# Farofeiro231/LiDAR_SLAM

Measured on AMD Instinct MI355X. Metric: scans/sec (RANSAC+UKF, 720-pt scans) at 1/2/4/8 MI355X + HBM GB/s vs peak, higher is better.
Workload: dtype f64; 1 GPU; C3: 4096 synthetic 720-pt scans per GPU, chunked 7x100+20; RANSAC (100 trials, 20 mm, mt19937 hypotheses) + landmark association + UKF predict/update (n=3, L=20); scans_per_gpu=4096, trials=100, landmarks=20, hyp=mt19937, parallelism=dp1 (scan shards, no collective)

## Files before the change

lidar_slam_amd/csrc/lslam_ctx.h:

```cpp
#pragma once
#include "lslam_hazards.h"

constexpr int LSLAM_EV_RING = 64;
constexpr int NSLOTS = 2;

static thread_local std::string g_err;

static size_t default_steps_budget() { return (size_t)2 << 30; }

static size_t default_reloc_budget() {
    if (const char *e = getenv("LSLAM_RELOC_BUDGET")) {
        const long long v = atoll(e);
        if (v > 0) return (size_t)v;
    }
    return (size_t)4096 * 41 * 21 * 21 * 4;
}

static int set_err(int code, const char *msg) {
    g_err = msg;
    return code;
}

#define HIPCHK(expr)                                                                  \
    do {                                                                              \
        hipError_t _e = (expr);                                                       \
        if (_e != hipSuccess) {                                                       \
            g_err = std::string(#expr) + ": " + hipGetErrorString(_e);                \
            return LSLAM_ERR_HIP;                                                     \
        }                                                                             \
    } while (0)

struct DevBuf {
    void *p = nullptr;
    size_t bytes = 0;
    template <typename T>
    T *as() const { return (T *)p; }
    hipError_t release() {
        void *q = p;
        p = nullptr;
        bytes = 0;
        return q ? hipFree(q) : hipSuccess;
    }
    static bool fits(const DevBuf *b, int n, size_t need) {
        for (int i = 0; i < n; i++)
            if (b[i].bytes < need) return false;
        return true;
    }
    static int ensure(lslam_ctx *c, DevBuf *b, int n, size_t need, const char *what);
    int ensure(lslam_ctx *c, size_t need, const char *what) { return ensure(c, this, 1, need, what); }
};

struct lslam_ctx {
    int device = 0;
    hipStream_t stream = nullptr;
    bool timing = false;
    hipEvent_t ev0[LSLAM_K_COUNT][LSLAM_EV_RING] = {}, ev1[LSLAM_K_COUNT][LSLAM_EV_RING] = {};
    int head[LSLAM_K_COUNT] = {}, npend[LSLAM_K_COUNT] = {};
    double total_ms[LSLAM_K_COUNT] = {};
    int64_t launches[LSLAM_K_COUNT] = {};
    DevBuf scr;
    DevBuf escr;
    DevBuf cscr;
    DevBuf mscr;
    DevBuf rscr;
    size_t reloc_budget = default_reloc_budget();
    int resolve_beside = 0;
    int n_cus = 1;
    uint32_t timing_mask = 0xffffffffu;
    uint32_t *rt_all = nullptr;
    DevBuf seedst[3];
    hipStream_t sstream = nullptr;
    hipEvent_t ev_seeded[2] = {};
    hipEvent_t ev_seed_read[2] = {};
    int seed_next = 0;
    DevBuf cutb[4];
    int cut_next = 0;
    size_t steps_budget = default_steps_budget();
    hipStream_t pstream = nullptr;
    DevBuf pslot[NSLOTS];
    int next_slot = 0;
    hipEvent_t ev_slot_free[NSLOTS] = {};
    hipEvent_t ev_produced = nullptr;
    hipEvent_t ev_copy = nullptr;
    hipEvent_t ev_call = nullptr;
    hipStream_t ustream = nullptr;
    hipEvent_t ev_ukf = nullptr;
    HazardState hz;
    int prev_slot = 0;
    DevBuf spec_dirty[2];
    int spec_cur = 0;
};

int DevBuf::ensure(lslam_ctx *c, DevBuf *b, int n, size_t need, const char *what) {
    if (fits(b, n, need)) return LSLAM_OK;
    for (hipStream_t s : {c->stream, c->pstream, c->ustream, c->sstream}) HIPCHK(hipStreamSynchronize(s));
    for (int i = 0; i < n; i++) HIPCHK(b[i].release());
    for (int i = 0; i < n; i++) {
        const hipError_t e = hipMalloc(&b[i].p, need);
        if (e == hipErrorOutOfMemory) {
            g_err = std::string("hipMalloc: out of memory (") + what + ")";
            return LSLAM_ERR_NOMEM;
        }
        HIPCHK(e);
        b[i].bytes = need;
    }
    return LSLAM_OK;
}

static const std::vector<uint32_t> &reject_tables() {
    static const std::vector<uint32_t> t = [] {
        std::vector<uint32_t> v((size_t)(RT_KMAX - 1) * RT_DWORDS);
        for (uint32_t K = 2; K <= RT_KMAX; K++)
            for (uint32_t r = 0; r < (uint32_t)RT_ROWS; r++)
                for (uint32_t q = 0; q < (uint32_t)RT_ST; q++)
                    v[(size_t)(K - 2) * RT_DWORDS + r * RT_ST + q] = rt_word(K, r, q);
        return v;
    }();
    return t;
}

static int ctx_init(lslam_ctx *c, int device) {
    c->device = device;
    HIPCHK(hipDeviceGetAttribute(&c->n_cus, hipDeviceAttributeMultiprocessorCount, device));
    if (c->n_cus < 1) c->n_cus = 1;
    if (const char *e = getenv("LSLAM_MT_SPECULATE")) c->hz.speculate = atoi(e) != 0;
    HIPCHK(hipStreamCreateWithFlags(&c->stream, hipStreamNonBlocking));
    for (int k = 0; k < LSLAM_K_COUNT; k++)
        for (int r = 0; r < LSLAM_EV_RING; r++) {
            HIPCHK(hipEventCreate(&c->ev0[k][r]));
            HIPCHK(hipEventCreate(&c->ev1[k][r]));
        }
    {
        int lo_pri = 0, hi_pri = 0;
        if (hipDeviceGetStreamPriorityRange(&lo_pri, &hi_pri) != hipSuccess) hi_pri = 0;
        HIPCHK(hipStreamCreateWithPriority(&c->pstream, hipStreamNonBlocking, hi_pri));
    }
    HIPCHK(hipStreamCreateWithFlags(&c->sstream, hipStreamNonBlocking));
    for (int i = 0; i < 2; i++) {
        HIPCHK(hipEventCreateWithFlags(&c->ev_seeded[i], hipEventDisableTiming));
        HIPCHK(hipEventCreateWithFlags(&c->ev_seed_read[i], hipEventDisableTiming));
        HIPCHK(hipEventRecord(c->ev_seed_read[i], c->stream));
    }
    for (int i = 0; i < NSLOTS; i++) HIPCHK(hipEventCreateWithFlags(&c->ev_slot_free[i], hipEventDisableTiming));
    HIPCHK(hipEventCreateWithFlags(&c->ev_produced, hipEventDisableTiming));
    HIPCHK(hipStreamCreateWithFlags(&c->ustream, hipStreamNonBlocking));
    HIPCHK(hipEventCreateWithFlags(&c->ev_ukf, hipEventDisableTiming));
    HIPCHK(hipEventCreateWithFlags(&c->ev_copy, hipEventDisableTiming));
    HIPCHK(hipEventCreateWithFlags(&c->ev_call, hipEventDisableTiming));
    for (int i = 0; i < NSLOTS; i++) HIPCHK(hipEventRecord(c->ev_slot_free[i], c->stream));
    HIPCHK(hipEventRecord(c->ev_copy, c->stream));
    HIPCHK(hipEventRecord(c->ev_call, c->stream));
    const std::vector<uint32_t> &t = reject_tables();
    HIPCHK(hipMalloc(&c->rt_all, t.size() * 4));
    HIPCHK(hipMemcpy(c->rt_all, t.data(), t.size() * 4, hipMemcpyHostToDevice));
    return LSLAM_OK;
}

extern "C" {

#define LSLAM_STR_(x) #x
#define LSLAM_STR(x) LSLAM_STR_(x)
#ifndef LSLAM_SRC_HASH
#define LSLAM_SRC_HASH "0000000000000000"
#endif
const char *lslam_version(void) {
    return "lidarslam-mi355x 0.3.0 (abi " LSLAM_STR(LSLAM_ABI_VERSION) ", src " LSLAM_SRC_HASH ", gfx950)";
}

const char *lslam_status_string(int st) {
    switch (st) {
        case LSLAM_OK: return "ok";
        case LSLAM_ERR_ARG: return "invalid argument";
        case LSLAM_ERR_HIP: return "HIP runtime error";
        case LSLAM_ERR_NOMEM: return "out of memory";
        case LSLAM_ERR_CAPACITY: return "capacity exceeded";
        case LSLAM_ERR_UNSUPPORTED: return "unsupported";
        default: return "unknown status";
    }
}

const char *lslam_last_error(void) { return g_err.c_str(); }

int lslam_device_count(int *n) {
    if (!n) return LSLAM_ERR_ARG;
    int c = 0;
    hipError_t e = hipGetDeviceCount(&c);
    if (e != hipSuccess) c = 0;
    *n = c;
    return LSLAM_OK;
}

int lslam_ctx_create(int device, lslam_ctx **out) {
    if (!out) return LSLAM_ERR_ARG;
    *out = nullptr;
    int n = 0;
    HIPCHK(hipGetDeviceCount(&n));
    if (device < 0 || device >= n) return set_err(LSLAM_ERR_ARG, "device index out of range");
    HIPCHK(hipSetDevice(device));
    lslam_ctx *c = new (std::nothrow) lslam_ctx();
    if (!c) return LSLAM_ERR_NOMEM;
    const int st = ctx_init(c, device);
    if (st) {
        lslam_ctx_destroy(c);
        return st;
    }
    *out = c;
    return LSLAM_OK;
}

int lslam_ctx_destroy(lslam_ctx *c) {
    if (!c) return LSLAM_OK;
    (void)hipSetDevice(c->device);
    hipStream_t streams[4] = {c->stream, c->pstream, c->ustream, c->sstream};
    for (hipStream_t s : streams)
        if (s) (void)hipStreamSynchronize(s);
    for (int k = 0; k < LSLAM_K_COUNT; k++)
        for (int r = 0; r < LSLAM_EV_RING; r++) {
            if (c->ev0[k][r]) (void)hipEventDestroy(c->ev0[k][r]);
            if (c->ev1[k][r]) (void)hipEventDestroy(c->ev1[k][r]);
        }
    for (DevBuf *b : {&c->scr, &c->escr, &c->cscr, &c->mscr, &c->rscr}) (void)b->release();
    for (DevBuf &b : c->seedst) (void)b.release();
    for (DevBuf &b : c->cutb) (void)b.release();
    for (DevBuf &b : c->pslot) (void)b.release();
    for (DevBuf &b : c->spec_dirty) (void)b.release();
    if (c->rt_all) (void)hipFree(c->rt_all);
    hipEvent_t evs[10] = {c->ev_seeded[0], c->ev_seeded[1], c->ev_seed_read[0], c->ev_seed_read[1], c->ev_slot_free[0],
                          c->ev_slot_free[1], c->ev_produced, c->ev_copy, c->ev_call, c->ev_ukf};
    for (hipEvent_t e : evs)
        if (e) (void)hipEventDestroy(e);
    for (hipStream_t s : streams)
        if (s) (void)hipStreamDestroy(s);
    delete c;
    return LSLAM_OK;
}

int lslam_sync(lslam_ctx *c) {
    if (!c) return LSLAM_ERR_ARG;
    HIPCHK(hipSetDevice(c->device));
    HIPCHK(hipStreamSynchronize(c->pstream));
    HIPCHK(hipStreamSynchronize(c->ustream));
    HIPCHK(hipStreamSynchronize(c->sstream));
    HIPCHK(hipStreamSynchronize(c->stream));
    return LSLAM_OK;
}

int lslam_malloc(lslam_ctx *c, size_t bytes, void **p) {
    if (!c || !p) return LSLAM_ERR_ARG;
    HIPCHK(hipSetDevice(c->device));
    *p = nullptr;
    if (bytes == 0) bytes = 16;
    hipError_t e = hipMalloc(p, bytes);
    if (e == hipErrorOutOfMemory) return set_err(LSLAM_ERR_NOMEM, "hipMalloc: out of memory");
    HIPCHK(e);
    return LSLAM_OK;
}

int lslam_free(lslam_ctx *c, void *p) {
    if (!c) return LSLAM_ERR_ARG;
    if (!p) return LSLAM_OK;
    HIPCHK(hipSetDevice(c->device));
    HIPCHK(hipFree(p));
    return LSLAM_OK;
}

int lslam_host_alloc(size_t bytes, void **p) {
    if (!p) return LSLAM_ERR_ARG;
    HIPCHK(hipHostMalloc(p, bytes ? bytes : 16, hipHostMallocDefault));
    return LSLAM_OK;
}

int lslam_host_free(void *p) {
    if (p) HIPCHK(hipHostFree(p));
    return LSLAM_OK;
}

int lslam_h2d(lslam_ctx *c, void *dst, const void *src, size_t n) {
    if (!c || (!dst && n) || (!src && n)) return LSLAM_ERR_ARG;
    if (!n) return LSLAM_OK;
    HIPCHK(hipSetDevice(c->device));
    HIPCHK(hipMemcpyAsync(dst, src, n, hipMemcpyHostToDevice, c->stream));
    HIPCHK(hipEventRecord(c->ev_copy, c->stream));
    c->hz.copies.add(dst, n);
    return LSLAM_OK;
}

int lslam_d2h(lslam_ctx *c, void *dst, const void *src, size_t n) {
    if (!c || (!dst && n) || (!src && n)) return LSLAM_ERR_ARG;
    if (!n) return LSLAM_OK;
    HIPCHK(hipSetDevice(c->device));
    HIPCHK(hipMemcpyAsync(dst, src, n, hipMemcpyDeviceToHost, c->stream));
    return LSLAM_OK;
}

int lslam_d2d(lslam_ctx *c, void *dst, const void *src, size_t n) {
    if (!c || (!dst && n) || (!src && n)) return LSLAM_ERR_ARG;
    if (!n) return LSLAM_OK;
    HIPCHK(hipSetDevice(c->device));
    HIPCHK(hipMemcpyAsync(dst, src, n, hipMemcpyDeviceToDevice, c->stream));
    HIPCHK(hipEventRecord(c->ev_copy, c->stream));
    c->hz.copies.add(dst, n);
    return LSLAM_OK;
}

int lslam_host_register(void *p, size_t n) {
    if (!p || !n) return LSLAM_ERR_ARG;
    const hipError_t e = hipHostRegister(p, n, hipHostRegisterDefault);
    if (e != hipSuccess) {
        (void)hipGetLastError();
        return set_err(LSLAM_ERR_HIP, hipGetErrorString(e));
    }
    return LSLAM_OK;
}

int lslam_host_unregister(void *p) {
    if (!p) return LSLAM_ERR_ARG;
    HIPCHK(hipHostUnregister(p));
    return LSLAM_OK;
}

int lslam_ctx_stream(lslam_ctx *c, void **stream) {
    if (!c || !stream) return LSLAM_ERR_ARG;
    *stream = (void *)c->stream;
    return LSLAM_OK;
}

int lslam_abi_sizes(int64_t *sizes, int n) {
    const int64_t s[9] = {(int64_t)sizeof(lslam_chunk_model), (int64_t)sizeof(lslam_landmark),
                          (int64_t)sizeof(lslam_ransac_params), (int64_t)sizeof(lslam_ukf_params),
                          (int64_t)sizeof(lslam_scan_batch), (int64_t)sizeof(lslam_express_measures),
                          (int64_t)sizeof(lslam_express_revs), (int64_t)sizeof(lslam_match_params),
                          (int64_t)sizeof(lslam_match_batch)};
    for (int i = 0; i < n && i < 9 && sizes; i++) sizes[i] = s[i];
    return 9;
}

int lslam_grid_abi_sizes(int64_t *sizes, int n) {
    const int64_t s[2] = {(int64_t)sizeof(lslam_grid_params), (int64_t)sizeof(lslam_grid_batch)};
    for (int i = 0; i < n && i < 2 && sizes; i++) sizes[i] = s[i];
    return 2;
}

int lslam_mapmatch_abi_sizes(int64_t *sizes, int n) {
    const int64_t s[2] = {(int64_t)sizeof(lslam_mapmatch_params), (int64_t)sizeof(lslam_mapmatch_batch)};
    for (int i = 0; i < n && i < 2 && sizes; i++) sizes[i] = s[i];
    return 2;
}

int lslam_mapfuse_abi_sizes(int64_t *sizes, int n) {
    const int64_t s[2] = {(int64_t)sizeof(lslam_mapfuse_params), (int64_t)sizeof(lslam_mapfuse_batch)};
    for (int i = 0; i < n && i < 2 && sizes; i++) sizes[i] = s[i];
    return 2;
}

int lslam_reloc_abi_sizes(int64_t *sizes, int n) {
    const int64_t s[2] = {(int64_t)sizeof(lslam_reloc_params), (int64_t)sizeof(lslam_reloc_batch)};
    for (int i = 0; i < n && i < 2 && sizes; i++) sizes[i] = s[i];
    return 2;
}

int lslam_raycast_abi_sizes(int64_t *sizes, int n) {
    const int64_t s[2] = {(int64_t)sizeof(lslam_raycast_params), (int64_t)sizeof(lslam_raycast_batch)};
    for (int i = 0; i < n && i < 2 && sizes; i++) sizes[i] = s[i];
    return 2;
}

int lslam_recentre_abi_sizes(int64_t *sizes, int n) {
    const int64_t s[2] = {(int64_t)sizeof(lslam_recentre_params), (int64_t)sizeof(lslam_recentre_batch)};
    for (int i = 0; i < n && i < 2 && sizes; i++) sizes[i] = s[i];
    return 2;
}

int lslam_dist_abi_sizes(int64_t *sizes, int n) {
    const int64_t s[4] = {(int64_t)sizeof(lslam_dist_params), (int64_t)sizeof(lslam_dist_batch),
                          (int64_t)sizeof(lslam_fieldscore_params), (int64_t)sizeof(lslam_fieldscore_batch)};
    for (int i = 0; i < n && i < 4 && sizes; i++) sizes[i] = s[i];
    return 4;
}

int lslam_memset(lslam_ctx *c, void *dst, int v, size_t n) {
    if (!c || (!dst && n)) return LSLAM_ERR_ARG;
    if (!n) return LSLAM_OK;
    HIPCHK(hipSetDevice(c->device));
    HIPCHK(hipMemsetAsync(dst, v, n, c->stream));
    HIPCHK(hipEventRecord(c->ev_copy, c->stream));
    c->hz.copies.add(dst, n);
    return LSLAM_OK;
}

static int harvest(lslam_ctx *c, int k, int upto_free = -1) {
    while (c->npend[k] > 0 && (upto_free < 0 || LSLAM_EV_RING - c->npend[k] < upto_free)) {
        const int r = (c->head[k] - c->npend[k] + LSLAM_EV_RING) % LSLAM_EV_RING;
        HIPCHK(hipEventSynchronize(c->ev1[k][r]));
        float ms = 0.f;
        HIPCHK(hipEventElapsedTime(&ms, c->ev0[k][r], c->ev1[k][r]));
        c->total_ms[k] += ms;
        c->launches[k] += 1;
        c->npend[k] -= 1;
    }
    return LSLAM_OK;
}

static int timer_begin(lslam_ctx *c, int k, hipStream_t st_ = nullptr) {
    if (!c->timing || !((c->timing_mask >> k) & 1u)) return LSLAM_OK;
    int st = harvest(c, k, 1);
    if (st) return st;
    HIPCHK(hipEventRecord(c->ev0[k][c->head[k]], st_ ? st_ : c->stream));
    return LSLAM_OK;
}

static int timer_end(lslam_ctx *c, int k, hipStream_t st_ = nullptr) {
    if (!c->timing || !((c->timing_mask >> k) & 1u)) return LSLAM_OK;
    HIPCHK(hipEventRecord(c->ev1[k][c->head[k]], st_ ? st_ : c->stream));
    c->head[k] = (c->head[k] + 1) % LSLAM_EV_RING;
    c->npend[k] += 1;
    return LSLAM_OK;
}

int lslam_set_timing(lslam_ctx *c, int en) {
    if (!c) return LSLAM_ERR_ARG;
    c->timing = en != 0;
    return LSLAM_OK;
}

int lslam_set_timing_mask(lslam_ctx *c, uint32_t mask) {
    if (!c) return LSLAM_ERR_ARG;
    c->timing_mask = mask;
    return LSLAM_OK;
}

int lslam_timing(lslam_ctx *c, int k, double *ms, int64_t *n) {
    if (!c || k < 0 || k >= LSLAM_K_COUNT) return LSLAM_ERR_ARG;
    HIPCHK(hipSetDevice(c->device));
    int st = harvest(c, k);
    if (st) return st;
    if (ms) *ms = c->total_ms[k];
    if (n) *n = c->launches[k];
    return LSLAM_OK;
}

int lslam_timing_reset(lslam_ctx *c) {
    if (!c) return LSLAM_ERR_ARG;
    for (int k = 0; k < LSLAM_K_COUNT; k++) {
        int st = harvest(c, k);
        if (st) return st;
        c->total_ms[k] = 0;
        c->launches[k] = 0;
    }
    return LSLAM_OK;
}

int lslam_ransac_params_default(lslam_ransac_params *p) {
    if (!p) return LSLAM_ERR_ARG;
    memset(p, 0, sizeof(*p));
    p->residual_threshold = 20.0;
    p->max_trials = 100;
    p->min_samples = 2;
    p->hyp_source = LSLAM_HYP_MT19937;
    p->life = 40;
    p->tol_a = 0.1;
    p->tol_b = 10.0;
    p->tol_dist = 100.0;
    p->philox_seed = 0x5eed5eedull;
    return LSLAM_OK;
}

int lslam_ukf_params_default(lslam_ukf_params *p, int32_t L) {
    if (!p || L < 0) return LSLAM_ERR_ARG;
    memset(p, 0, sizeof(*p));
// ... 145 lines not shown
```

lidar_slam_amd/csrc/lslam_hazards.h:

```cpp
#pragma once
#include <stddef.h>
#include <stdint.h>

#include "../../include/lidarslam.h"

constexpr int LSLAM_MAX_COPIES = 32;
constexpr int LSLAM_MAX_OUTS = 48;
constexpr int SPEC_RESYNC = 32;

static inline bool ranges_overlap(const void *a, size_t na, const void *b, size_t nb) {
    if (!a || !b || !na || !nb) return false;
    const uintptr_t x = (uintptr_t)a, y = (uintptr_t)b;
    return x < y + nb && y < x + na;
}

template <int CAP>
struct RangeSet {
    struct { const void *p; size_t n; } r[CAP];
    int n = 0;
    bool overflow = false;
    void add(const void *p, size_t len) {
        if (!p || !len) return;
        for (int i = 0; i < n; i++)
            if (r[i].p == p && r[i].n == len) return;
        if (n == CAP) {
            overflow = true;
            return;
        }
        r[n].p = p;
        r[n].n = len;
        n++;
    }
    bool hits(const void *p, size_t len) const {
        if (overflow) return true;
        for (int i = 0; i < n; i++)
            if (ranges_overlap(p, len, r[i].p, r[i].n)) return true;
        return false;
    }
    void clear() {
        n = 0;
        overflow = false;
    }
};

struct ProducerInputs {
    const void *p[4];
    size_t n[4];
    enum { SEEDS, SCAN_CHUNK_OFF, CHUNK_PT_OFF, MT_STATE_IN };
};
static inline ProducerInputs producer_inputs(const lslam_scan_batch *b) {
    return {{b->seeds, b->scan_chunk_off, b->chunk_pt_off, b->mt_state_in},
            {(size_t)b->n_scans * 4, (size_t)(b->n_scans + 1) * 4, (size_t)(b->n_chunks + 1) * 4,
             (size_t)b->n_scans * 625 * 4}};
}

struct HazardState {
    RangeSet<LSLAM_MAX_COPIES> copies;
    RangeSet<LSLAM_MAX_OUTS> outs;
    const void *prev_state_out = nullptr;
    int prev_fixed = 0;
    int speculate = 1;
    int spec_ok = 0;
    int spec_run = 0;
    const uint32_t *prev_state_scr = nullptr;
    int prev_spec_scans = 0;
};

struct ProducerPlan {
    bool wait_copy;
    int hazard;
    bool spec;
    bool wait_prev_slot;
    bool resolve_beside;
};

static inline ProducerPlan plan_producer(HazardState &h, const lslam_scan_batch *b, int ep_count) {
    const ProducerInputs in = producer_inputs(b);
    ProducerPlan pl;
    const bool state_copied = h.copies.hits(in.p[ProducerInputs::MT_STATE_IN], in.n[ProducerInputs::MT_STATE_IN]);
    pl.wait_copy = false;
    for (int i = 0; i < 4; i++) pl.wait_copy |= h.copies.hits(in.p[i], in.n[i]);
    if (pl.wait_copy) h.copies.clear();
    pl.hazard = h.outs.overflow ? 2 : 0;
    for (int i = 0; i < 4 && !h.outs.overflow; i++)
        for (int j = 0; j < h.outs.n; j++)
            if (ranges_overlap(in.p[i], in.n[i], h.outs.r[j].p, h.outs.r[j].n)) {
                const bool chained = i == ProducerInputs::MT_STATE_IN && h.outs.r[j].p == h.prev_state_out && h.prev_fixed;
                if (pl.hazard < 2) pl.hazard = chained ? 1 : 2;
            }
    if (pl.hazard == 2) h.outs.clear();
    pl.spec = pl.hazard == 1 && h.speculate && h.spec_ok && ep_count == 1 && h.prev_state_scr &&
              h.prev_spec_scans == b->n_scans && b->mt_state_in == h.prev_state_out && !state_copied;
    if (pl.spec && ++h.spec_run >= SPEC_RESYNC) pl.spec = false;
    if (!pl.spec) h.spec_run = 0;
    pl.wait_prev_slot = pl.hazard == 1 && !pl.spec;
    pl.resolve_beside = pl.hazard == 0 || pl.spec;
    return pl;
}
```

lidar_slam_amd/csrc/lslam_launch.h:

```cpp
#pragma once
#include <type_traits>

static inline int align16(int x) { return (x + 15) & ~15; }

template <typename F>
static void with_hyp_source(int hyp_source, F &&f) {
    switch (hyp_source) {
        case LSLAM_HYP_PHILOX: f(std::integral_constant<int, LSLAM_HYP_PHILOX>{}); break;
        case LSLAM_HYP_EXPLICIT: f(std::integral_constant<int, LSLAM_HYP_EXPLICIT>{}); break;
        default: f(std::integral_constant<int, LSLAM_HYP_MT19937>{}); break;
    }
}

static int validate_batch(const lslam_scan_batch *b, bool need_points) {
    if (!b) return set_err(LSLAM_ERR_ARG, "batch is NULL");
    if (b->n_scans < 0 || b->n_chunks < 0 || b->n_points < 0) return set_err(LSLAM_ERR_ARG, "negative sizes");
    if (b->n_scans == 0) return LSLAM_OK;
    if (!b->scan_chunk_off || !b->chunk_pt_off) return set_err(LSLAM_ERR_ARG, "missing CSR offsets");
    if (need_points && !b->xy && (!b->theta_deg || !b->dist_mm) && b->n_points > 0)
        return set_err(LSLAM_ERR_ARG, "missing points (xy, or theta_deg + dist_mm)");
    if (b->max_chunk_points < 0 || b->max_scan_chunks < 0) return set_err(LSLAM_ERR_ARG, "bad maxima");
    return LSLAM_OK;
}

// ... 209 lines not shown
    const size_t budget = c->steps_budget;
    const int D = k.T + 1;
    int De = D;
    if (k.b.max_scan_chunks == 1 && (size_t)D * per_draw > budget) {
        const size_t fit = budget / per_draw;
        De = fit < 1 ? 1 : (fit < (size_t)D ? (int)fit : D);
    }
    k.ep_nd = De < D ? De : 0;
    k.ep_d0 = 0;
    k.ep_count = (D + De - 1) / De;
    const size_t jbytes = ((size_t)De * per_draw + JBUF_FRONT + 64 + 255) & ~(size_t)255;
    const size_t sbytes = ((size_t)(k.b.n_scans > 0 ? k.b.n_scans : 1) * 625 * 4 + 255) & ~(size_t)255;
    if (!DevBuf::fits(c->pslot, NSLOTS, jbytes + sbytes)) c->hz.spec_ok = 0;
    int st = DevBuf::ensure(c, c->pslot, NSLOTS, jbytes + sbytes, "producer slot");
    if (st) return st;
    k.jbuf = c->pslot[slot].as<unsigned char>() + JBUF_FRONT;
    k.state_scr = (uint32_t *)(c->pslot[slot].as<unsigned char>() + jbytes);
    k.slot_jbytes = jbytes;
    if (k.b.draws_out) {
        k.draws_scr = k.b.draws_out;
    } else {
        st = c->scr.ensure(c, (size_t)(k.b.n_chunks > 0 ? k.b.n_chunks : 1) * 2 * (k.T + 1) * 4, "step scratch");
        if (st) return st;
        k.draws_scr = c->scr.as<int32_t>();
    }
    return LSLAM_OK;
}

static int launch_resolve(lslam_ctx *c, const KArgs &base, hipStream_t rs) {
    if (base.b.n_chunks == 0) return LSLAM_OK;
    KArgs k = base;
    const int N = k.b.max_chunk_points > 3 ? k.b.max_chunk_points : 3;
    const int esz = k.j8 ? 1 : 2;
    const int De = k.ep_nd > 0 ? k.ep_nd : k.T + 1;
    const int64_t need = ((int64_t)De * (N - 1) * esz + 46) & ~(int64_t)15;
    const int lds = need <= 16 * 1024 ? (int)need : 0;
    k.res_g = lds;
    if (lds == 0) {
        const int64_t items = (int64_t)k.b.n_chunks * De;
        const int64_t cap = k.ep_count > 1 ? 16 * (int64_t)c->n_cus : (1 << 20);
        const dim3 grid(launch_cap(items > cap ? cap : items)), block(64);
        if (k.j8) hipLaunchKernelGGL((resolve_walk_kernel<uint8_t, 16>), grid, block, 0, rs, k);
        else hipLaunchKernelGGL((resolve_walk_kernel<uint16_t, 16>), grid, block, 0, rs, k);
        HIPCHK(hipGetLastError());
        return LSLAM_OK;
    }
    if (k.j8 && c->resolve_beside) {
        if (N - 1 <= 16 * RR_GROUPS - 1) {
            const bool has_last = k.ep_d0 + De == k.T + 1;
            const int Dres = (has_last && !k.b.draws_out && De > 1) ? De - 1 : De;
            if ((int64_t)k.b.n_chunks * Dres >= ((int64_t)1 << 31) - 64)
                return set_err(LSLAM_ERR_UNSUPPORTED, "more than 2^31 chunk draws in one call");
            const dim3 grid(launch_cap(((int64_t)k.b.n_chunks * Dres + 63) / 64)), block(64);
            hipLaunchKernelGGL(resolve_reg8_kernel, grid, block, 0, rs, k, Dres);
        } else {
            const dim3 grid(launch_cap(k.b.n_chunks)), block(64);
            hipLaunchKernelGGL(resolve_reg_kernel, grid, block, 0, rs, k);
        }
        HIPCHK(hipGetLastError());
        return LSLAM_OK;
    }
    static std::once_flag once;
    std::call_once(once, [] {
        set_max_lds(resolve_kernel<uint8_t>);
        set_max_lds(resolve_kernel<uint16_t>);
    });
    const dim3 grid(launch_cap(k.b.n_chunks)), block(64);
    if (k.j8) hipLaunchKernelGGL(resolve_kernel<uint8_t>, grid, block, lds, rs, k);
    else hipLaunchKernelGGL(resolve_kernel<uint16_t>, grid, block, lds, rs, k);
    HIPCHK(hipGetLastError());
    return LSLAM_OK;
}

static int launch_seed(lslam_ctx *c, KArgs &k, hipStream_t ss, int i) {
    int st = c->seedst[i].ensure(c, (size_t)k.b.n_scans * MT_N * 4, "seed states");
    if (st) return st;
    hipLaunchKernelGGL(seed_kernel, dim3((unsigned)((k.b.n_scans + 63) / 64)), dim3(64), 0, ss, k.b.seeds,
                       (int)k.b.n_scans, c->seedst[i].as<uint32_t>());
    HIPCHK(hipGetLastError());
    k.seed_state = c->seedst[i].as<uint32_t>();
    return LSLAM_OK;
}

static int launch_cuts(lslam_ctx *c, KArgs &k, hipStream_t ss) {
    k.cuts = nullptr;
    if (k.b.n_chunks <= 0 || k.b.max_chunk_points > 128) return LSLAM_OK;
    DevBuf &cb = c->cutb[c->cut_next];
    int st = cb.ensure(c, (size_t)k.b.n_chunks * sizeof(ChunkCut), "chunk cutoffs");
    if (st) return st;
    hipLaunchKernelGGL(cut_lane_kernel, dim3((unsigned)((k.b.n_chunks + 63) / 64)), dim3(64), 0, ss, k, cb.as<ChunkCut>());
    HIPCHK(hipGetLastError());
    k.cuts = cb.as<ChunkCut>();
    c->cut_next = (c->cut_next + 1) & 3;
    return LSLAM_OK;
}

static int seed_beside(lslam_ctx *c, KArgs &k, const ProducerPlan &pl, int &buf) {
    buf = -1;
    if (k.b.mt_state_in) return LSLAM_OK;
    const int i = c->seed_next;
    hipStream_t ss = c->sstream;
    HIPCHK(hipStreamWaitEvent(ss, c->ev_seed_read[i], 0));
    if (pl.wait_copy) HIPCHK(hipStreamWaitEvent(ss, c->ev_copy, 0));
    if (pl.hazard == 2) HIPCHK(hipStreamWaitEvent(ss, c->ev_call, 0));
    int st = launch_seed(c, k, ss, i);
    if (st) return st;
    if ((st = launch_cuts(c, k, ss))) return st;
    HIPCHK(hipEventRecord(c->ev_seeded[i], ss));
    HIPCHK(hipStreamWaitEvent(c->pstream, c->ev_seeded[i], 0));
    c->seed_next ^= 1;
    buf = i;
    return LSLAM_OK;
}

static int launch_rng(lslam_ctx *c, const KArgs &base, hipStream_t stream) {
    KArgs k = base;
    k.rt_all = c->rt_all;
    if (k.b.mt_state_in || k.ep_d0 != 0) k.seed_state = nullptr;
    int lds = 0;
    int st = layout_rng(k, &k.b, lds);
    if (st) return st;
    static std::once_flag once;
    std::call_once(once, [] {
        set_max_lds(rng_kernel<uint8_t>);
        set_max_lds(rng_kernel<uint16_t>);
    });
    st = timer_begin(c, LSLAM_K_RNG, stream);
    if (st) return st;
    const dim3 grid((unsigned)((k.b.n_scans + RNG_PPW - 1) / RNG_PPW)), block(64 * RNG_PPW);
    if (k.j8) hipLaunchKernelGGL((rng_kernel<uint8_t>), grid, block, lds, stream, k);
    else hipLaunchKernelGGL((rng_kernel<uint16_t>), grid, block, lds, stream, k);
    HIPCHK(hipGetLastError());
    return timer_end(c, LSLAM_K_RNG, stream);
}

static int produce_draws(lslam_ctx *c, KArgs &k, int slot, hipStream_t ps, uint32_t *final_out, int &last_slot) {
    const int D = k.T + 1;
    const uint32_t *prev_state = nullptr;
    int sl = slot;
    for (int e = 0; e < k.ep_count; e++) {
        KArgs ke = k;
        if (k.ep_count > 1) {
            ke.ep_d0 = e * k.ep_nd;
            ke.ep_nd = std::min(k.ep_nd, D - ke.ep_d0);
            ke.jbuf = c->pslot[sl].as<unsigned char>() + JBUF_FRONT;
            ke.state_scr = (uint32_t *)(c->pslot[sl].as<unsigned char>() + k.slot_jbytes);
            if (e > 0) {
                if (ps != c->stream) HIPCHK(hipStreamWaitEvent(ps, c->ev_slot_free[sl], 0));
                ke.b.mt_state_in = prev_state;
            }
        }
        const bool last = e == k.ep_count - 1;
        ke.b.mt_state_out = (last && final_out) ? final_out : ke.state_scr;
        int st = launch_rng(c, ke, ps);
        if (st) return st;
        if (ps != c->stream) {
            HIPCHK(hipEventRecord(c->ev_produced, ps));
            HIPCHK(hipStreamWaitEvent(c->stream, c->ev_produced, 0));
        }
        st = launch_resolve(c, ke, c->stream);
        if (st) return st;
        if (!last) HIPCHK(hipEventRecord(c->ev_slot_free[sl], c->stream));
        prev_state = ke.state_scr;
        last_slot = sl;
        sl = (sl + 1) % NSLOTS;
    }
    k.state_scr = const_cast<uint32_t *>(prev_state);
    c->next_slot = sl;
    return LSLAM_OK;
}

static void remember_outputs(lslam_ctx *c, const lslam_scan_batch *b, int T, int L) {
    const size_t S = (size_t)b->n_scans, C = (size_t)b->n_chunks, P = (size_t)b->n_points;
    const void *p[11] = {b->inlier_mask, b->models, b->y_proj, b->draws_out, b->trial_cnt_out, b->mt_state_out,
                         b->landmarks, b->lmk_count, b->lmk_walk, b->ukf_x, b->ukf_P};
    const size_t n[11] = {P, C * sizeof(lslam_chunk_model), P * 8, C * 2 * (T + 1) * 4, C * T * 4, S * 625 * 4,
                          S * b->lmk_capacity * sizeof(lslam_landmark), S * 4, S * b->lmk_capacity * 4,
                          L ? S * 24 : 0, L ? S * 72 : 0};
    for (int i = 0; i < 11; i++) c->hz.outs.add(p[i], n[i]);
}

static int mark_calls(lslam_ctx *c) {
    HIPCHK(hipEventRecord(c->ev_call, c->stream));
    return LSLAM_OK;
}

static int layout_select(KArgs &k, const lslam_scan_batch *b, int &lds) {
    const int N = b->max_chunk_points > 0 ? b->max_chunk_points : 1;
    const int T = k.T > 0 ? k.T : 1;
    int off = 0;
    k.off_pts = off; off += align16(16 * N);
    k.off_tied = off; off += align16(4 * T);
// ... 38 lines not shown
        hipLaunchKernelGGL(model_kernel<decltype(H)::value>, mgrid, block, 0, c->stream, k);
    });
    HIPCHK(hipGetLastError());
    if (k.cnt_blocks > 0) {
        const dim3 grid((unsigned)(nc * k.cnt_blocks)), cblock(CNT_TPB);
        if (N <= 256) hipLaunchKernelGGL(count_kernel<1>, grid, cblock, 0, c->stream, k);
        else if (N <= 512) hipLaunchKernelGGL(count_kernel<2>, grid, cblock, 0, c->stream, k);
        else if (N <= 1024) hipLaunchKernelGGL(count_kernel<4>, grid, cblock, 0, c->stream, k);
        else if (N <= 2048) hipLaunchKernelGGL(count_kernel<8>, grid, cblock, 0, c->stream, k);
        else hipLaunchKernelGGL(count_kernel<16>, grid, cblock, 0, c->stream, k);
        HIPCHK(hipGetLastError());
    }
    const dim3 grid((unsigned)nc), sblock(64);
    with_hyp_source(k.hyp_source, [&](auto H) {
        hipLaunchKernelGGL(select_kernel<decltype(H)::value>, grid, sblock, lds_sel, c->stream, k);
    });
    HIPCHK(hipGetLastError());
    return LSLAM_OK;
}

static int launch_chunks(lslam_ctx *c, const KArgs &base, bool write_yproj) {
    if (base.b.n_chunks == 0) return LSLAM_OK;
    KArgs k = base;
    k.write_yproj = write_yproj ? 1 : 0;
    int st = timer_begin(c, LSLAM_K_CONSENSUS);
    if (st) return st;
    if (k.b.max_chunk_points > 128) {
        st = launch_chunks_large(c, k);
        if (st) return st;
        return timer_end(c, LSLAM_K_CONSENSUS);
    }
    int lds = 0;
    st = layout_chunk(k, &k.b, lds);
    if (st) return st;
    static std::once_flag once;
    std::call_once(once, [] {
        set_max_lds(chunk_kernel<LSLAM_HYP_MT19937>);
        set_max_lds(chunk_kernel<LSLAM_HYP_PHILOX>);
        set_max_lds(chunk_kernel<LSLAM_HYP_EXPLICIT>);
    });
    const dim3 grid(launch_cap(k.b.n_chunks)), block(64);
    with_hyp_source(k.hyp_source, [&](auto H) {
        hipLaunchKernelGGL(chunk_kernel<decltype(H)::value>, grid, block, lds, c->stream, k);
    });
    HIPCHK(hipGetLastError());
    return timer_end(c, LSLAM_K_CONSENSUS);
}

template <int MODE>
static int launch_post(lslam_ctx *c, const KArgs &k, int lds) {
    static std::once_flag once;
    std::call_once(once, [] {
        set_max_lds(scan_kernel<LSLAM_HYP_EXPLICIT, MODE>);
        set_max_lds(scan_kernel_w4<LSLAM_HYP_EXPLICIT, MODE>);
    });
    const dim3 grid(launch_cap(k.b.n_scans));
    if (MODE == MODE_ASSOC && k.lmk_reg) {
        static std::once_flag once_reg;
        std::call_once(once_reg, [] { set_max_lds(post_reg_kernel); });
        hipLaunchKernelGGL(post_reg_kernel, grid, dim3(64), lds, c->stream, k);
    } else if (k.hyp_source == LSLAM_HYP_MT19937)
        hipLaunchKernelGGL((scan_kernel<LSLAM_HYP_EXPLICIT, MODE>), grid, dim3(64), lds, c->stream, k);
    else
        hipLaunchKernelGGL((scan_kernel_w4<LSLAM_HYP_EXPLICIT, MODE>), grid, dim3(64), lds, c->stream, k);
    HIPCHK(hipGetLastError());
    return LSLAM_OK;
}

static int run_split(lslam_ctx *c, const lslam_scan_batch *b, const lslam_ransac_params *p,
                     const lslam_ukf_params *u) {
    HIPCHK(hipSetDevice(c->device));
    if (b->n_scans == 0) return LSLAM_OK;
#if defined(LSLAM_STAMPS) || defined(LSLAM_CENSUS)
    g_call_seq += 1;
#endif
    const bool assoc = b->landmarks != nullptr;
    KArgs k;
    int lds_fix = 0;
    int st = build_args(k, b, p, nullptr, MODE_RANSAC, lds_fix);
    if (st) return st;
    const bool mt = k.hyp_source == LSLAM_HYP_MT19937;
    bool spec = false;
    int seed_buf = -1;
    int slot = c->next_slot;
    if (mt) {
        st = prepare_steps(c, k, slot);
        if (st) return st;
        c->next_slot = (c->next_slot + 1) % NSLOTS;
    }
    KArgs kp;
    int lds_post = 0;
    const bool ukf_side = p->hyp_source != LSLAM_HYP_MT19937 && u &&
                          !(u->flags & (LSLAM_UKF_LMK_FROM_RANSAC | LSLAM_UKF_MAP));
    const bool ukf_lane = u && !ukf_side && !(u->flags & LSLAM_UKF_MAP);
    const int pmode = (assoc ? MODE_ASSOC : MODE_POST) | (u && !ukf_side && !ukf_lane ? MODE_UKF : 0);
    if ((pmode & MODE_UKF) && !(u->flags & LSLAM_UKF_MAP))
        return set_err(LSLAM_ERR_UNSUPPORTED, "post pass given a non-map UKF step");
    if (assoc || (u && !ukf_side && !ukf_lane)) {
        st = build_args(kp, b, p, (ukf_side || ukf_lane) ? nullptr : u, pmode, lds_post);
        if (st) return st;
    }
    KArgs kl;
    if (ukf_lane) {
        int lds_l = 0;
        st = build_args(kl, b, p, u, MODE_UKF, lds_l);
        if (st) return st;
        if ((u->flags & LSLAM_UKF_LMK_FROM_RANSAC) && !b->models)
            return set_err(LSLAM_ERR_ARG, "LSLAM_UKF_LMK_FROM_RANSAC needs the chunk models");
    }
    KArgs ku;
    int lds_u = 0;
    if (ukf_side) {
        st = build_args(ku, b, nullptr, u, MODE_UKF, lds_u);
        if (st) return st;
    }
    st = timer_begin(c, LSLAM_K_PIPELINE);
    if (st) return st;
    if (ukf_side) {
        if ((st = mark_calls(c))) return st;
        HIPCHK(hipStreamWaitEvent(c->ustream, c->ev_call, 0));
        HIPCHK(hipStreamWaitEvent(c->ustream, c->ev_copy, 0));
        launch_ukf_group(ku, u->n_landmarks, c->ustream, false);
        HIPCHK(hipGetLastError());
        HIPCHK(hipEventRecord(c->ev_ukf, c->ustream));
    }
    if (mt) {
        const ProducerPlan pl = plan_producer(c->hz, b, k.ep_count);
        if (pl.wait_copy) HIPCHK(hipStreamWaitEvent(c->pstream, c->ev_copy, 0));
        if (pl.hazard == 2) {
            if ((st = mark_calls(c))) return st;
            HIPCHK(hipStreamWaitEvent(c->pstream, c->ev_call, 0));
        }
        if ((st = seed_beside(c, k, pl, seed_buf))) return st;
        HIPCHK(hipStreamWaitEvent(c->pstream, c->ev_slot_free[slot], 0));
        spec = pl.spec;
        if (pl.wait_prev_slot) HIPCHK(hipStreamWaitEvent(c->pstream, c->ev_slot_free[c->prev_slot], 0));
        c->resolve_beside = pl.resolve_beside;
        const uint32_t *true_in = k.b.mt_state_in;
        if (spec) k.b.mt_state_in = c->hz.prev_state_scr;
        st = produce_draws(c, k, slot, c->pstream, nullptr, slot);
        k.b.mt_state_in = true_in;
        if (st) return st;
        if (seed_buf >= 0) HIPCHK(hipEventRecord(c->ev_seed_read[seed_buf], c->pstream));
    }
    const bool ukf_indep = ukf_lane && !(u->flags & (LSLAM_UKF_LMK_FROM_RANSAC | LSLAM_UKF_MAP));
    st = launch_chunks(c, k, !assoc);
    if (st) return st;
    if (mt) {
        KArgs kf = k;
        kf.fixup = 1;
        if (k.ep_count == 1 && b->mt_state_out) {
            if (spec && !DevBuf::fits(c->spec_dirty, 2, (size_t)b->n_scans))
                return set_err(LSLAM_ERR_HIP, "speculation without replay flags");
            if ((st = DevBuf::ensure(c, c->spec_dirty, 2, (size_t)b->n_scans, "flags"))) return st;
            kf.spec_dirty_in = spec ? c->spec_dirty[c->spec_cur].as<uint8_t>() : nullptr;
            kf.spec_dirty_out = c->spec_dirty[c->spec_cur ^ 1].as<uint8_t>();
        }
        static std::once_flag once;
        std::call_once(once, [] { set_max_lds(scan_kernel<LSLAM_HYP_MT19937, MODE_RANSAC>); });
        hipLaunchKernelGGL((scan_kernel<LSLAM_HYP_MT19937, MODE_RANSAC>), dim3(launch_cap(b->n_scans)), dim3(64), lds_fix,
                           c->stream, kf);
        HIPCHK(hipGetLastError());
        HIPCHK(hipEventRecord(c->ev_slot_free[slot], c->stream));
    }
    if (ukf_indep) {
        launch_ukf_group(kl, u->n_landmarks, c->stream, true);
        HIPCHK(hipGetLastError());
    }
    c->hz.prev_state_out = mt ? b->mt_state_out : nullptr;
    c->prev_slot = slot;
    c->hz.prev_fixed = mt ? 1 : 0;
    c->hz.spec_ok = (mt && k.ep_count == 1 && b->mt_state_out) ? 1 : 0;
    if (c->hz.spec_ok) {
        c->spec_cur ^= 1;
        c->hz.prev_state_scr = k.state_scr;
        c->hz.prev_spec_scans = b->n_scans;
    }
    switch (pmode) {
        case MODE_ASSOC | MODE_UKF: st = launch_post<MODE_ASSOC | MODE_UKF>(c, kp, lds_post); break;
        case MODE_POST | MODE_UKF: st = launch_post<MODE_POST | MODE_UKF>(c, kp, lds_post); break;
        case MODE_ASSOC: st = launch_post<MODE_ASSOC>(c, kp, lds_post); break;
        default: break;
    }
    if (st) return st;
    if (ukf_lane && !ukf_indep) {
        launch_ukf_group(kl, u->n_landmarks, c->stream, true);
        HIPCHK(hipGetLastError());
    }
    if (ukf_side) HIPCHK(hipStreamWaitEvent(c->stream, c->ev_ukf, 0));
    remember_outputs(c, b, k.T, u ? u->n_landmarks : 0);
    return timer_end(c, LSLAM_K_PIPELINE);
}



static int corr_check_params(const char *who, const char *width_name, double theta_step, int width, int smear, int k_trans,
                             int k_theta) {
    const std::string p = std::string(who) + ": ";
    if (!(theta_step > 0) || !std::isfinite(theta_step)) return set_err(LSLAM_ERR_ARG, (p + "theta_step must be > 0").c_str());
    if (width < 16 || width > 512 || (width & 1))
        return set_err(LSLAM_ERR_ARG, (p + width_name + " must be even, in [16, 512]").c_str());
    if (smear < 0 || smear > 2) return set_err(LSLAM_ERR_ARG, (p + "smear must be in [0, 2]").c_str());
    if (k_trans < 0 || k_trans > 15) return set_err(LSLAM_ERR_ARG, (p + "k_trans must be in [0, 15]").c_str());
    if (k_theta < 0 || k_theta > 31) return set_err(LSLAM_ERR_ARG, (p + "k_theta must be in [0, 31]").c_str());
    return LSLAM_OK;
}

static int corr_geometry(lslam_ctx *c, const char *who, int n, double cell, double theta_step, int width, int smear,
                         int k_trans, int k_theta, int32_t *scores, CorrGeom &g, size_t &vol) {
    g.cell = cell;
    g.inv = 1.0 / cell;
    g.theta_step = theta_step;
    g.n = n;
    g.win_w = width;
    g.half = width / 2;
    g.smear = smear;
    g.kt = k_trans;
    g.kth = k_theta;
    g.Nt = 2 * k_trans + 1;
    g.Nth = 2 * k_theta + 1;
    g.W = width + 2 * k_trans;
    g.Sd = match_row_dwords(g.W);
    const int64_t want = 2 * (int64_t)c->n_cus;
    int64_t ns = (want + n - 1) / n;
    ns = std::min<int64_t>(std::max<int64_t>(ns, 1), g.Nth);
    g.per_slice = (int)((g.Nth + ns - 1) / ns);
    g.n_slices = (g.Nth + g.per_slice - 1) / g.per_slice;
    if ((int64_t)n * g.n_slices >= ((int64_t)1 << 31))
// ... 860 lines not shown
    if (!c) return set_err(LSLAM_ERR_ARG, "fieldscore: ctx is NULL");
    if (b->n_robots == 0) return LSLAM_OK;
    HIPCHK(hipSetDevice(c->device));
    return launch_fieldscore(c, b, g, p);
}

int lslam_set_reloc_budget(lslam_ctx *c, int64_t bytes) {
    if (!c) return LSLAM_ERR_ARG;
    c->reloc_budget = bytes > 0 ? (size_t)bytes : default_reloc_budget();
    return LSLAM_OK;
}

int lslam_express_decode(lslam_ctx *c, const uint8_t *packets, int64_t n_packets, const lslam_express_measures *out) {
    if (!c || !out) return LSLAM_ERR_ARG;
    int st = express_check(packets, n_packets);
    if (st) return st;
    if (n_packets == 0) return LSLAM_OK;
    HIPCHK(hipSetDevice(c->device));
    ExpressOut o{out->angle_deg, out->dist_mm, out->new_scan, out->valid, (double2 *)out->xy, out->pkt_valid};
    if ((st = timer_begin(c, LSLAM_K_EXPRESS))) return st;
    const int64_t blocks = (n_packets + EXP_DEC_PER_WG - 1) / EXP_DEC_PER_WG;
    hipLaunchKernelGGL(express_decode_kernel, dim3((unsigned)blocks), dim3(256), 0, c->stream, packets, n_packets, o);
    HIPCHK(hipGetLastError());
    if ((st = timer_end(c, LSLAM_K_EXPRESS))) return st;
    const size_t nm = (size_t)(n_packets > 1 ? n_packets - 1 : 0) * 32;
    c->hz.outs.add(out->angle_deg, nm * 8);
    c->hz.outs.add(out->dist_mm, nm * 8);
    c->hz.outs.add(out->new_scan, nm);
    c->hz.outs.add(out->valid, nm);
    c->hz.outs.add(out->xy, nm * 16);
    c->hz.outs.add(out->pkt_valid, (size_t)n_packets);
    return LSLAM_OK;
}

int lslam_express_scans(lslam_ctx *c, const uint8_t *packets, int64_t n_packets, int32_t skip,
                        const lslam_express_revs *out) {
    if (!c || !out || !out->counts || !out->scan_chunk_off || !out->chunk_pt_off) return LSLAM_ERR_ARG;
    if (out->cap_scans < 0 || out->cap_chunks < 0 || out->cap_points < 0 || (out->cap_points > 0 && !out->xy))
        return set_err(LSLAM_ERR_ARG, "express: bad output capacities");
    int st = express_check(packets, n_packets);
    if (st) return st;
    if (skip < 0 || skip > 31) return set_err(LSLAM_ERR_ARG, "express: skip must be in [0, 31]");
    HIPCHK(hipSetDevice(c->device));
    const int64_t np = n_packets > 1 ? n_packets - 1 : 0;
    const int64_t tiles = (np + EXP_TILE - 1) / EXP_TILE;
    size_t off = 0;
    const size_t o_flags = off;
    off = align256(off + (size_t)np);
    const size_t o_tile = off;
    off = align256(off + (size_t)tiles * sizeof(int2));
    const size_t o_rank = off;
    off = align256(off + (size_t)np * sizeof(int2));
    const size_t o_rend = off;
    off = align256(off + (size_t)np * sizeof(int2));
    const size_t o_rinfo = off;
    off = align256(off + (size_t)np * sizeof(int4));
    if ((st = c->escr.ensure(c, off > 0 ? off : 256, "express scratch"))) return st;
    uint8_t *base = c->escr.as<uint8_t>();
    ExpressScratch s{base + o_flags, (int2 *)(base + o_tile), (int2 *)(base + o_rank), (int2 *)(base + o_rend),
                     (int4 *)(base + o_rinfo), out->counts};
    ExpressScans o{(double2 *)out->xy, out->scan_chunk_off, out->chunk_pt_off, out->cap_points, out->cap_scans,
                   out->cap_chunks};
    if ((st = timer_begin(c, LSLAM_K_EXPRESS))) return st;
    if (tiles > 0) {
        hipLaunchKernelGGL(express_flags_kernel, dim3((unsigned)tiles), dim3(256), 0, c->stream, packets, n_packets,
                           (int)skip, s);
        HIPCHK(hipGetLastError());
        hipLaunchKernelGGL(express_rank_kernel, dim3((unsigned)tiles), dim3(256), 0, c->stream, n_packets, (int)skip, s);
        HIPCHK(hipGetLastError());
    }
    hipLaunchKernelGGL(express_revs_kernel, dim3((unsigned)(tiles > 0 ? tiles : 1)), dim3(256), 0, c->stream,
                       (int)tiles, s, o);
    HIPCHK(hipGetLastError());
    if (np > 0) {
        if ((st = timer_begin(c, LSLAM_K_EXPRESS_SCATTER))) return st;
        const int64_t blocks = (np + EXP_DEC_PER_WG - 1) / EXP_DEC_PER_WG;
        hipLaunchKernelGGL(express_scatter_kernel, dim3((unsigned)blocks), dim3(256), 0, c->stream, packets, n_packets,
                           (int)skip, s, o);
        HIPCHK(hipGetLastError());
        if ((st = timer_end(c, LSLAM_K_EXPRESS_SCATTER))) return st;
    }
    if ((st = timer_end(c, LSLAM_K_EXPRESS))) return st;
    HIPCHK(hipEventRecord(c->ev_copy, c->stream));
    c->hz.copies.add(out->xy, (size_t)out->cap_points * 16);
    c->hz.copies.add(out->scan_chunk_off, ((size_t)out->cap_scans + 1) * 4);
    c->hz.copies.add(out->chunk_pt_off, ((size_t)out->cap_chunks + 1) * 4);
    c->hz.copies.add(out->counts, 16);
    return LSLAM_OK;
}

}
```

Baseline: 6.263 million scans/s.

## Track point-input copy hazards for chunk-cut precompute on side stream

Adds a separate copy-range set for point inputs (xy, theta, dist) so the chunk-cutoff precompute on the seed stream can wait on pending copies, or fall back to in-kernel cuts when point data is a prior output. Previously the cut kernel ran on the side stream without any ordering against host copies of point data. When a wait is needed, the cut launch is moved after seeding and the main stream waits on a new ev_cuts event. This is mostly a correctness fix for a race, with a small extra event and wait added in the hazardous case.

```diff
diff --git a/lidar_slam_amd/csrc/lslam_ctx.h b/lidar_slam_amd/csrc/lslam_ctx.h
--- a/lidar_slam_amd/csrc/lslam_ctx.h
+++ b/lidar_slam_amd/csrc/lslam_ctx.h
@@ -72,6 +72,7 @@
     hipStream_t sstream = nullptr;
     hipEvent_t ev_seeded[2] = {};
     hipEvent_t ev_seed_read[2] = {};
+    hipEvent_t ev_cuts = nullptr;
     int seed_next = 0;
     DevBuf cutb[4];
     int cut_next = 0;
@@ -143,6 +144,7 @@
     }
     for (int i = 0; i < NSLOTS; i++) HIPCHK(hipEventCreateWithFlags(&c->ev_slot_free[i], hipEventDisableTiming));
     HIPCHK(hipEventCreateWithFlags(&c->ev_produced, hipEventDisableTiming));
+    HIPCHK(hipEventCreateWithFlags(&c->ev_cuts, hipEventDisableTiming));
     HIPCHK(hipStreamCreateWithFlags(&c->ustream, hipStreamNonBlocking));
     HIPCHK(hipEventCreateWithFlags(&c->ev_ukf, hipEventDisableTiming));
     HIPCHK(hipEventCreateWithFlags(&c->ev_copy, hipEventDisableTiming));
@@ -225,8 +227,8 @@
     for (DevBuf &b : c->pslot) (void)b.release();
     for (DevBuf &b : c->spec_dirty) (void)b.release();
     if (c->rt_all) (void)hipFree(c->rt_all);
-    hipEvent_t evs[10] = {c->ev_seeded[0], c->ev_seeded[1], c->ev_seed_read[0], c->ev_seed_read[1], c->ev_slot_free[0],
-                          c->ev_slot_free[1], c->ev_produced, c->ev_copy, c->ev_call, c->ev_ukf};
+    hipEvent_t evs[11] = {c->ev_seeded[0], c->ev_seeded[1], c->ev_seed_read[0], c->ev_seed_read[1], c->ev_slot_free[0],
+                          c->ev_slot_free[1], c->ev_produced, c->ev_copy, c->ev_call, c->ev_ukf, c->ev_cuts};
     for (hipEvent_t e : evs)
         if (e) (void)hipEventDestroy(e);
     for (hipStream_t s : streams)
@@ -281,7 +283,7 @@
     HIPCHK(hipSetDevice(c->device));
     HIPCHK(hipMemcpyAsync(dst, src, n, hipMemcpyHostToDevice, c->stream));
     HIPCHK(hipEventRecord(c->ev_copy, c->stream));
-    c->hz.copies.add(dst, n);
+    c->hz.note_copy(dst, n);
     return LSLAM_OK;
 }
 
@@ -299,7 +301,7 @@
     HIPCHK(hipSetDevice(c->device));
     HIPCHK(hipMemcpyAsync(dst, src, n, hipMemcpyDeviceToDevice, c->stream));
     HIPCHK(hipEventRecord(c->ev_copy, c->stream));
-    c->hz.copies.add(dst, n);
+    c->hz.note_copy(dst, n);
     return LSLAM_OK;
 }
 
@@ -384,7 +386,7 @@
     HIPCHK(hipSetDevice(c->device));
     HIPCHK(hipMemsetAsync(dst, v, n, c->stream));
     HIPCHK(hipEventRecord(c->ev_copy, c->stream));
-    c->hz.copies.add(dst, n);
+    c->hz.note_copy(dst, n);
     return LSLAM_OK;
 }
 
diff --git a/lidar_slam_amd/csrc/lslam_hazards.h b/lidar_slam_amd/csrc/lslam_hazards.h
--- a/lidar_slam_amd/csrc/lslam_hazards.h
+++ b/lidar_slam_amd/csrc/lslam_hazards.h
@@ -53,9 +53,22 @@
             {(size_t)b->n_scans * 4, (size_t)(b->n_scans + 1) * 4, (size_t)(b->n_chunks + 1) * 4,
              (size_t)b->n_scans * 625 * 4}};
 }
+struct PointInputs {
+    const void *p[3];
+    size_t n[3];
+};
+static inline PointInputs point_inputs(const lslam_scan_batch *b) {
+    const size_t P = (size_t)b->n_points;
+    return {{b->xy, b->theta_deg, b->dist_mm}, {P * 16, P * 8, P * 8}};
+}
 
 struct HazardState {
     RangeSet<LSLAM_MAX_COPIES> copies;
+    RangeSet<LSLAM_MAX_COPIES> pt_copies;
+    void note_copy(const void *p, size_t len) {
+        copies.add(p, len);
+        pt_copies.add(p, len);
+    }
     RangeSet<LSLAM_MAX_OUTS> outs;
     const void *prev_state_out = nullptr;
     int prev_fixed = 0;
@@ -72,6 +85,8 @@
     bool spec;
     bool wait_prev_slot;
     bool resolve_beside;
+    bool cuts_wait_copy;
+    bool cuts_in_kernel;
 };
 
 static inline ProducerPlan plan_producer(HazardState &h, const lslam_scan_batch *b, int ep_count) {
@@ -81,6 +96,15 @@
     pl.wait_copy = false;
     for (int i = 0; i < 4; i++) pl.wait_copy |= h.copies.hits(in.p[i], in.n[i]);
     if (pl.wait_copy) h.copies.clear();
+    const bool cuts = !b->mt_state_in && b->n_chunks > 0 && b->max_chunk_points <= 128;
+    const PointInputs pts = point_inputs(b);
+    pl.cuts_wait_copy = pl.cuts_in_kernel = false;
+    for (int i = 0; i < 3 && cuts; i++) {
+        pl.cuts_wait_copy |= h.pt_copies.hits(pts.p[i], pts.n[i]);
+        pl.cuts_in_kernel |= h.outs.hits(pts.p[i], pts.n[i]);
+    }
+    if (cuts && (pl.wait_copy || pl.cuts_wait_copy)) h.pt_copies.clear();
+    if (pl.wait_copy) pl.cuts_wait_copy = false;
     pl.hazard = h.outs.overflow ? 2 : 0;
     for (int i = 0; i < 4 && !h.outs.overflow; i++)
         for (int j = 0; j < h.outs.n; j++)
@@ -95,5 +119,6 @@
     if (!pl.spec) h.spec_run = 0;
     pl.wait_prev_slot = pl.hazard == 1 && !pl.spec;
     pl.resolve_beside = pl.hazard == 0 || pl.spec;
+    if (pl.hazard == 2) pl.cuts_in_kernel = false;
     return pl;
 }
diff --git a/lidar_slam_amd/csrc/lslam_launch.h b/lidar_slam_amd/csrc/lslam_launch.h
--- a/lidar_slam_amd/csrc/lslam_launch.h
+++ b/lidar_slam_amd/csrc/lslam_launch.h
@@ -315,9 +315,10 @@
     return LSLAM_OK;
 }
 
-static int launch_cuts(lslam_ctx *c, KArgs &k, hipStream_t ss) {
+static int launch_cuts(lslam_ctx *c, KArgs &k, hipStream_t ss, const ProducerPlan &pl, bool &cuts_waited) {
     k.cuts = nullptr;
-    if (k.b.n_chunks <= 0 || k.b.max_chunk_points > 128) return LSLAM_OK;
+    if (k.b.n_chunks <= 0 || k.b.max_chunk_points > 128 || pl.cuts_in_kernel) return LSLAM_OK;
+    if (pl.cuts_wait_copy) HIPCHK(hipStreamWaitEvent(ss, c->ev_copy, 0));
     DevBuf &cb = c->cutb[c->cut_next];
     int st = cb.ensure(c, (size_t)k.b.n_chunks * sizeof(ChunkCut), "chunk cutoffs");
     if (st) return st;
@@ -325,11 +326,16 @@
     HIPCHK(hipGetLastError());
     k.cuts = cb.as<ChunkCut>();
     c->cut_next = (c->cut_next + 1) & 3;
-    return LSLAM_OK;
-}
-
-static int seed_beside(lslam_ctx *c, KArgs &k, const ProducerPlan &pl, int &buf) {
+    if (pl.cuts_wait_copy) {
+        HIPCHK(hipEventRecord(c->ev_cuts, ss));
+        cuts_waited = true;
+    }
+    return LSLAM_OK;
+}
+
+static int seed_beside(lslam_ctx *c, KArgs &k, const ProducerPlan &pl, int &buf, bool &cuts_waited) {
     buf = -1;
+    cuts_waited = false;
     if (k.b.mt_state_in) return LSLAM_OK;
     const int i = c->seed_next;
     hipStream_t ss = c->sstream;
@@ -338,9 +344,10 @@
     if (pl.hazard == 2) HIPCHK(hipStreamWaitEvent(ss, c->ev_call, 0));
     int st = launch_seed(c, k, ss, i);
     if (st) return st;
-    if ((st = launch_cuts(c, k, ss))) return st;
+    if (!pl.cuts_wait_copy && (st = launch_cuts(c, k, ss, pl, cuts_waited))) return st;
     HIPCHK(hipEventRecord(c->ev_seeded[i], ss));
     HIPCHK(hipStreamWaitEvent(c->pstream, c->ev_seeded[i], 0));
+    if (pl.cuts_wait_copy && (st = launch_cuts(c, k, ss, pl, cuts_waited))) return st;
     c->seed_next ^= 1;
     buf = i;
     return LSLAM_OK;
@@ -545,6 +552,7 @@
     const bool mt = k.hyp_source == LSLAM_HYP_MT19937;
     bool spec = false;
     int seed_buf = -1;
+    bool cuts_waited = false;
     int slot = c->next_slot;
     if (mt) {
         st = prepare_steps(c, k, slot);
@@ -594,7 +602,7 @@
             if ((st = mark_calls(c))) return st;
             HIPCHK(hipStreamWaitEvent(c->pstream, c->ev_call, 0));
         }
-        if ((st = seed_beside(c, k, pl, seed_buf))) return st;
+        if ((st = seed_beside(c, k, pl, seed_buf, cuts_waited))) return st;
         HIPCHK(hipStreamWaitEvent(c->pstream, c->ev_slot_free[slot], 0));
         spec = pl.spec;
         if (pl.wait_prev_slot) HIPCHK(hipStreamWaitEvent(c->pstream, c->ev_slot_free[c->prev_slot], 0));
@@ -607,6 +615,7 @@
         if (seed_buf >= 0) HIPCHK(hipEventRecord(c->ev_seed_read[seed_buf], c->pstream));
     }
     const bool ukf_indep = ukf_lane && !(u->flags & (LSLAM_UKF_LMK_FROM_RANSAC | LSLAM_UKF_MAP));
+    if (cuts_waited) HIPCHK(hipStreamWaitEvent(c->stream, c->ev_cuts, 0));
     st = launch_chunks(c, k, !assoc);
     if (st) return st;
     if (mt) {
@@ -1633,11 +1642,11 @@
     }
     if ((st = timer_end(c, LSLAM_K_EXPRESS))) return st;
     HIPCHK(hipEventRecord(c->ev_copy, c->stream));
-    c->hz.copies.add(out->xy, (size_t)out->cap_points * 16);
-    c->hz.copies.add(out->scan_chunk_off, ((size_t)out->cap_scans + 1) * 4);
-    c->hz.copies.add(out->chunk_pt_off, ((size_t)out->cap_chunks + 1) * 4);
-    c->hz.copies.add(out->counts, 16);
-    return LSLAM_OK;
-}
-
-}
+    c->hz.note_copy(out->xy, (size_t)out->cap_points * 16);
+    c->hz.note_copy(out->scan_chunk_off, ((size_t)out->cap_scans + 1) * 4);
+    c->hz.note_copy(out->chunk_pt_off, ((size_t)out->cap_chunks + 1) * 4);
+    c->hz.note_copy(out->counts, 16);
+    return LSLAM_OK;
+}
+
+}
```

Result: no change. 6.264 million scans/s (median of 3 runs) (+0.0%).
